# kmaninis/OSVOS-PyTorch

Measured on NVIDIA H100. Metric: frames/sec at 480x854 fwd-only, batch 1 per GPU (OSVOS.forward -> 5 logit maps), higher is better.
Workload: dtype bf16x3 (split-bf16 operands, fp32 accumulate)

## Files before the change

### osvos_pytorch_b200/csrc/conv3x3_halo.cu

```cuda
#include <stdlib.h>
#include <string.h>

#include "conv_common.cuh"

namespace osvos {

constexpr int kHaloRows = kTileH + 2;

template <int BLOCK_N, int PLANES, int PITCH, bool SPLIT>
struct HaloCfg {
  static constexpr int kABoxBytes = kHaloRows * PITCH * 128;
  static constexpr int kAPlaneBytes = (kABoxBytes + 1023) / 1024 * 1024;
  static constexpr int kAStageBytes = PLANES * kAPlaneBytes;
  static constexpr int kAStages = 2;
  static constexpr int kBPlaneBytes = BLOCK_N * 128;
  static constexpr int kBStageBytes = PLANES * kBPlaneBytes;
  static constexpr int kBudget = 225 * 1024 - kAStages * kAStageBytes;
  static constexpr int kBStagesRaw = kBudget / kBStageBytes;
  static constexpr int kBStages = kBStagesRaw > 9 ? 9 : kBStagesRaw;
  static constexpr bool kSplitAcc = SPLIT;
  static_assert(!SPLIT || (PLANES == 2 && BLOCK_N <= 128), "split accumulators need two planes and 2 * BLOCK_N <= 256");
  static constexpr int kAccCols = kSplitAcc ? 2 * BLOCK_N : BLOCK_N;
  static constexpr int kAcc = kAccCols / 2;
  static constexpr int kSmemBytes = kAStages * kAStageBytes + kBStages * kBStageBytes + 1024 + 512;
  static_assert(kBStages >= 2, "weight ring too shallow");
  static_assert(kSmemBytes <= 227 * 1024, "more than the per-CTA shared memory of sm_90");
  static_assert(kSmemBytes + 4096 < (1 << 18), "descriptor start-address field would overflow");
  static_assert(kBStageBytes % 1024 == 0, "B stage must keep 1024-byte alignment");
};

template <int BLOCK_N, int PLANES, int PITCH, bool SPLIT, bool LEAN>
__global__ void __launch_bounds__(kConvThreads, 1)
conv3x3_halo_kernel(const __grid_constant__ CUtensorMap map_x_hi, const __grid_constant__ CUtensorMap map_x_lo,
                    const __grid_constant__ CUtensorMap map_w_hi, const __grid_constant__ CUtensorMap map_w_lo,
                    const ConvParams p) {
  using Cfg = HaloCfg<BLOCK_N, PLANES, PITCH, SPLIT>;
  constexpr int SA = Cfg::kAStages, SB = Cfg::kBStages;

  extern __shared__ uint8_t smem_raw[];
  uint8_t* smem = reinterpret_cast<uint8_t*>((reinterpret_cast<uintptr_t>(smem_raw) + 1023) & ~uintptr_t(1023));
  uint8_t* smem_a = smem;
  uint8_t* smem_b = smem + SA * Cfg::kAStageBytes;
  uint64_t* bars = reinterpret_cast<uint64_t*>(smem_b + SB * Cfg::kBStageBytes);
  uint64_t* a_full = bars;
  uint64_t* a_empty = bars + SA;
  uint64_t* b_full = bars + 2 * SA;
  uint64_t* b_empty = bars + 2 * SA + SB;

  const int warp = threadIdx.x >> 5;
  const int lane = threadIdx.x & 31;

  if (warp == 0 && lane == 0) {
    tma_prefetch_desc(&map_x_hi);
    tma_prefetch_desc(&map_w_hi);
    if (PLANES == 2) {
      tma_prefetch_desc(&map_x_lo);
      tma_prefetch_desc(&map_w_lo);
    }
    for (int i = 0; i < SA; ++i) {
      mbar_init(&a_full[i], 1);
      mbar_init(&a_empty[i], 2);
    }
    for (int i = 0; i < SB; ++i) {
      mbar_init(&b_full[i], 1);
      mbar_init(&b_empty[i], 2);
    }
    fence_barrier_init();
  }
  __syncthreads();
  pdl_wait();
  pdl_launch_dependents();

  if (warp == 0) {
    if (elect_one()) {
      int a_stage = 0, b_stage = 0;
      uint32_t a_phase = 0, b_phase = 0;
      const bool skip_a = (p.ablate & 2) != 0, skip_b = (p.ablate & 1) != 0;
      auto issue_a = [&](int x0, int y0, int img, int kc) {
        mbar_wait(&a_empty[a_stage], a_phase ^ 1);
        if (skip_a) {
          mbar_arrive(&a_full[a_stage]);
        } else {
          uint8_t* st = smem_a + a_stage * Cfg::kAStageBytes;
          mbar_arrive_expect_tx(&a_full[a_stage], PLANES * Cfg::kABoxBytes);
          tma_load_4d(&map_x_hi, &a_full[a_stage], st, kc * kBlockK, x0, y0, img);
          if (PLANES == 2) tma_load_4d(&map_x_lo, &a_full[a_stage], st + Cfg::kAPlaneBytes, kc * kBlockK, x0, y0, img);
        }
        if (++a_stage == SA) {
          a_stage = 0;
          a_phase ^= 1;
        }
      };
      int nb = 0, tx = 0, ty = 0, img = 0;
      const int w_first = static_cast<int>(blockIdx.x), w_stride = static_cast<int>(gridDim.x);
      if (w_first < p.total_tiles) {
        decode_tile(p, w_first, nb, tx, ty, img);
        issue_a(tx * kTileW - 1, ty * kTileH - 1, img, 0);
      }
      for (int tile = w_first; tile < p.total_tiles; tile += w_stride) {
        const bool has_next = tile + w_stride < p.total_tiles;
        int nnb = 0, ntx = 0, nty = 0, nimg = 0;
        if (has_next) decode_tile(p, tile + w_stride, nnb, ntx, nty, nimg);
        const int n0 = nb * BLOCK_N;
        for (int kc = 0; kc < p.k_chunks; ++kc) {
          const int c0 = kc * kBlockK;
#pragma unroll
          for (int tap = 0; tap < 9; ++tap) {
            if (tap == 3) {
              if (kc + 1 < p.k_chunks) issue_a(tx * kTileW - 1, ty * kTileH - 1, img, kc + 1);
              else if (has_next) issue_a(ntx * kTileW - 1, nty * kTileH - 1, nimg, 0);
            }
            mbar_wait(&b_empty[b_stage], b_phase ^ 1);
            if (skip_b) {
              mbar_arrive(&b_full[b_stage]);
            } else {
              uint8_t* st = smem_b + b_stage * Cfg::kBStageBytes;
              mbar_arrive_expect_tx(&b_full[b_stage], Cfg::kBStageBytes);
              tma_load_3d(&map_w_hi, &b_full[b_stage], st, c0, n0, tap);
              if (PLANES == 2) tma_load_3d(&map_w_lo, &b_full[b_stage], st + Cfg::kBPlaneBytes, c0, n0, tap);
            }
            if (++b_stage == SB) {
              b_stage = 0;
              b_phase ^= 1;
            }
          }
        }
        nb = nnb, tx = ntx, ty = nty, img = nimg;
      }
    }
    __syncwarp();
  } else if (warp >= 4) {
    const int wg = (warp - 4) >> 2, wl = warp & 3;
    const bool leader = (threadIdx.x & 127) == 0;
    constexpr uint64_t kDescA = desc_template(16, PITCH * 128, kDescSW128);
    constexpr uint64_t kDescB = desc_template(16, 1024, kDescSW128);
    constexpr uint32_t kLoPlaneA = Cfg::kAPlaneBytes >> 4, kLoPlaneB = Cfg::kBPlaneBytes >> 4;
    const uint32_t smem_a_u32 = smem_u32(smem_a) + wg * 8 * PITCH * 128, smem_b_u32 = smem_u32(smem_b);
    const int k_steps = (p.ablate & 4) ? 0 : p.k_steps;
    float acc[Cfg::kAcc];
    int a_stage = 0, b_stage = 0;
    uint32_t a_phase = 0, b_phase = 0;
    StageRelease pending;
    for (int tile = blockIdx.x; tile < p.total_tiles; tile += gridDim.x) {
#pragma unroll
      for (int i = 0; i < Cfg::kAcc; ++i) acc[i] = 0.f;
      for (int kc = 0; kc < p.k_chunks; ++kc) {
        mbar_wait(&a_full[a_stage], a_phase);
        const uint64_t da0 = kDescA | static_cast<uint64_t>((smem_a_u32 + a_stage * Cfg::kAStageBytes) >> 4);
#pragma unroll
        for (int tap = 0; tap < 9; ++tap) {
          const uint32_t tap_off = static_cast<uint32_t>(((tap / 3) * PITCH + (tap % 3)) * (128 >> 4));
          mbar_wait(&b_full[b_stage], b_phase);
          const uint64_t db_hi = kDescB | static_cast<uint64_t>((smem_b_u32 + b_stage * Cfg::kBStageBytes) >> 4);
          const uint64_t da_hi = da0 + tap_off;
          const uint64_t da_lo = da_hi + kLoPlaneA;
          wgmma_fence();
          auto k_step = [&](int k) {
            if constexpr (Cfg::kSplitAcc) {
              wgmma_bf16<2 * BLOCK_N>(acc, da_hi + 2 * k, db_hi + 2 * k, 1);
              wgmma_bf16<BLOCK_N>(acc, da_lo + 2 * k, db_hi + 2 * k, 1);
            } else if constexpr (PLANES == 2) {
              wgmma_bf16<BLOCK_N>(acc, da_lo + 2 * k, db_hi + 2 * k, 1);
              wgmma_bf16<BLOCK_N>(acc, da_hi + 2 * k, db_hi + kLoPlaneB + 2 * k, 1);
              wgmma_bf16<BLOCK_N>(acc, da_hi + 2 * k, db_hi + 2 * k, 1);
            } else {
              wgmma_bf16<BLOCK_N>(acc, da_hi + 2 * k, db_hi + 2 * k, 1);
            }
          };
          if (k_steps == kBlockK / 16) {
#pragma unroll
            for (int k = 0; k < kBlockK / 16; ++k) k_step(k);
          } else {
            for (int k = 0; k < k_steps; ++k) k_step(k);
          }
          wgmma_commit();
          wgmma_wait<1>();
          pending.release(leader);
          pending.bar_b = &b_empty[b_stage];
          if (tap == 8) pending.bar_a = &a_empty[a_stage];
          if (++b_stage == SB) {
            b_stage = 0;
            b_phase ^= 1;
          }
        }
        if (++a_stage == SA) {
          a_stage = 0;
          a_phase ^= 1;
        }
      }
      wgmma_wait<0>();
      wgmma_fence_operands(acc);
      pending.release(leader);
      conv_epilogue<BLOCK_N, Cfg::kSplitAcc, LEAN>(p, acc, tile, wg, wl, lane);
    }
  }
}

struct HaloSwitches {
  bool lean;
  bool n256;
  bool splitacc128;
};
static bool env_flag(const char* name, bool dflt) {
  const char* e = getenv(name);
  return e == nullptr ? dflt : atoi(e) != 0;
}
static HaloSwitches halo_switches() {
  static HaloSwitches sw;
  static int state = 0;
  if (state != 1) {
    sw.lean = env_flag("OSVOS_HALO_LEAN", true);
    sw.n256 = env_flag("OSVOS_CONV_N256", true);
    sw.splitacc128 = env_flag("OSVOS_SPLITACC128", true);
    state = env_flag("OSVOS_ENV_RELOAD", false) ? 2 : 1;
  }
  return sw;
}

template <int BLOCK_N, int PLANES, int PITCH, bool SPLIT = (PLANES == 2 && BLOCK_N <= 128), bool LEAN = false>
static int launch_halo(const osvos_conv3x3_args* a, cudaStream_t stream) {
  using Cfg = HaloCfg<BLOCK_N, PLANES, PITCH, SPLIT>;
  ConvParams p;
  fill_conv_params(p, a, BLOCK_N);
  const int sms = device_sm_count();
  CUtensorMap mx_hi, mx_lo, mw_hi, mw_lo;
  {
    const uint64_t dims[4] = {(uint64_t)a->cin, (uint64_t)a->w, (uint64_t)a->h, (uint64_t)a->n};
    const uint64_t strides[3] = {(uint64_t)a->cin * 2, (uint64_t)a->w * a->cin * 2,
                                 (uint64_t)a->h * a->w * a->cin * 2};
    const uint32_t box[4] = {kBlockK, PITCH, kHaloRows, 1};
    int rc = encode_tensor_map(&mx_hi, CU_TENSOR_MAP_DATA_TYPE_BFLOAT16, 2, 4, a->x_hi, dims, strides, box,
                               CU_TENSOR_MAP_SWIZZLE_128B);
    if (rc) return rc;
    rc = encode_tensor_map(&mx_lo, CU_TENSOR_MAP_DATA_TYPE_BFLOAT16, 2, 4, PLANES == 2 ? a->x_lo : a->x_hi, dims,
                           strides, box, CU_TENSOR_MAP_SWIZZLE_128B);
    if (rc) return rc;
  }
  int rc = encode_weight_maps(&mw_hi, &mw_lo, a, BLOCK_N);
  if (rc) return rc;
  auto kern = conv3x3_halo_kernel<BLOCK_N, PLANES, PITCH, SPLIT, LEAN>;
  static uint64_t attr_done = 0;
  OSVOS_CHECK_CUDA(ensure_dynamic_smem(kern, Cfg::kSmemBytes, &attr_done));
  const int grid = p.total_tiles < sms ? p.total_tiles : sms;
  OSVOS_CHECK_CUDA(launch_pdl(kern, dim3(grid), dim3(kConvThreads), Cfg::kSmemBytes, stream, mx_hi, mx_lo,
                              mw_hi, mw_lo, p));
  return OSVOS_OK;
}

template <int PITCH>
static int dispatch_halo(const osvos_conv3x3_args* a, cudaStream_t stream) {
  const bool fast = (a->flags & OSVOS_FLAG_FAST) != 0;
  const HaloSwitches sw = halo_switches();
  if (a->cout == 16) return fast ? launch_halo<16, 1, PITCH>(a, stream) : launch_halo<16, 2, PITCH>(a, stream);
  const bool lean = sw.lean && !fast && !(a->flags & OSVOS_FLAG_RELU_MASK) && a->colsum == nullptr && a->y_f32 == nullptr &&
                    a->pq == nullptr && a->k_valid == 0;
  if (a->cout == 64) {
    if (lean) return launch_halo<64, 2, PITCH, true, true>(a, stream);
    return fast ? launch_halo<64, 1, PITCH>(a, stream) : launch_halo<64, 2, PITCH>(a, stream);
  }
  const int m_tiles = ((a->w + kTileW - 1) / kTileW) * ((a->h + kTileH - 1) / kTileH) * a->n;
  const int sms = device_sm_count();
  const long tiles128 = static_cast<long>(m_tiles) * (a->cout / 128);
  const long waves128 = (tiles128 + sms - 1) / sms;
  const long waves256 = (static_cast<long>(m_tiles) * (a->cout / 256) + sms - 1) / sms;
  if (waves128 == 1 && tiles128 * 5 <= static_cast<long>(sms) * 3) {
    if (lean) return launch_halo<64, 2, PITCH, true, true>(a, stream);
    return fast ? launch_halo<64, 1, PITCH>(a, stream) : launch_halo<64, 2, PITCH>(a, stream);
  }
  const bool prefer256 = fast ? waves256 * 1100 < waves128 * 700 : waves256 * 2200 < waves128 * 1000;
  if (a->cout % 256 == 0 && prefer256 && sw.n256)
    return fast ? launch_halo<256, 1, PITCH>(a, stream) : launch_halo<256, 2, PITCH>(a, stream);
  if (fast) return launch_halo<128, 1, PITCH>(a, stream);
  if (!sw.splitacc128) return launch_halo<128, 2, PITCH, false>(a, stream);
  if (lean) return launch_halo<128, 2, PITCH, true, true>(a, stream);
  return launch_halo<128, 2, PITCH>(a, stream);
}

int conv3x3_halo_dispatch(const osvos_conv3x3_args* a, cudaStream_t stream) {
  return dispatch_halo<10>(a, stream);
}

static int check_conv_args(const osvos_conv3x3_args* a) {
  OSVOS_CHECK_ARG(a != nullptr);
  OSVOS_CHECK_ARG(a->n > 0 && a->h > 0 && a->w > 0);
  OSVOS_CHECK_ARG(a->cin >= 64 && a->cin % 64 == 0);
  OSVOS_CHECK_ARG(a->cout == 2 || a->cout == 16 || a->cout == 64 || (a->cout > 0 && a->cout % 128 == 0));
  OSVOS_CHECK_ARG(a->cout != 2 || (a->pq != nullptr && a->y_hi == nullptr && a->y_f32 == nullptr && a->pool_hi == nullptr &&
                                   a->colsum == nullptr && !(a->flags & (OSVOS_FLAG_RELU | OSVOS_FLAG_RELU_MASK)) &&
                                   a->k_valid == 0));
  OSVOS_CHECK_ARG(a->x_hi != nullptr && a->w_packed != nullptr);
  OSVOS_CHECK_ARG((a->flags & OSVOS_FLAG_FAST) || a->x_lo != nullptr);
  OSVOS_CHECK_ARG(a->y_hi != nullptr || a->y_f32 != nullptr || a->pq != nullptr || a->pool_hi != nullptr);
  OSVOS_CHECK_ARG(!(a->flags & OSVOS_FLAG_RELU_MASK) || a->mask_hi != nullptr);
  OSVOS_CHECK_ARG(a->pq == nullptr || a->cout == 2 || (a->cout == 16 && a->proj_w != nullptr));
  OSVOS_CHECK_ARG((a->pool_hi == nullptr && a->colsum == nullptr) || a->cout >= 64);
  OSVOS_CHECK_ARG((reinterpret_cast<uintptr_t>(a->x_hi) & 15) == 0);
  OSVOS_CHECK_ARG((reinterpret_cast<uintptr_t>(a->w_packed) & 15) == 0);
  OSVOS_CHECK_ARG((reinterpret_cast<uintptr_t>(a->bias) & 15) == 0);
  if (a->cout >= 64) {
    const uintptr_t bf16_planes = reinterpret_cast<uintptr_t>(a->y_hi) | reinterpret_cast<uintptr_t>(a->y_lo) |
                                  reinterpret_cast<uintptr_t>(a->pool_hi) | reinterpret_cast<uintptr_t>(a->pool_lo) |
                                  reinterpret_cast<uintptr_t>(a->mask_hi);
    OSVOS_CHECK_ARG((bf16_planes & 3) == 0);
    OSVOS_CHECK_ARG((reinterpret_cast<uintptr_t>(a->y_f32) & 7) == 0);
  }
  OSVOS_CHECK_ARG(a->k_valid >= 0 && a->k_valid <= 64 && a->k_valid % 16 == 0);
  return OSVOS_OK;
}

}

using namespace osvos;

extern "C" int osvos_side_folded_multi(const osvos_conv3x3_args* args, int count, osvos_stream_t stream_) {
  OSVOS_CHECK_ARG(args != nullptr && count > 0 && count <= 4);
  const osvos_conv3x3_args* order[4];
  for (int k = 0; k < count; ++k) {
    int rc = check_conv_args(&args[k]);
    if (rc) return rc;
    OSVOS_CHECK_ARG(args[k].cout == 2);
    OSVOS_CHECK_ARG((args[k].flags & OSVOS_FLAG_FAST) == (args[0].flags & OSVOS_FLAG_FAST));
    order[k] = &args[k];
  }
  for (int i = 1; i < count; ++i)
    for (int j = i; j > 0 && order[j]->cin > order[j - 1]->cin; --j) {
      const osvos_conv3x3_args* t = order[j];
      order[j] = order[j - 1];
      order[j - 1] = t;
    }
  return side_conv_multi_dispatch(order, count, static_cast<cudaStream_t>(stream_));
}

extern "C" int osvos_conv3x3(const osvos_conv3x3_args* a, osvos_stream_t stream_) {
  int rc = check_conv_args(a);
  if (rc) return rc;
  cudaStream_t stream = static_cast<cudaStream_t>(stream_);
  if (a->cout == 2) return side_conv_dispatch(a, stream);
  if (a->cout == 16 && a->y_hi == nullptr && !(a->flags & OSVOS_FLAG_RELU_MASK) && a->colsum == nullptr) {
    static int generic = -1;
    if (generic < 0) {
      const char* side = getenv("OSVOS_SIDE_IMPL");
      generic = (side != nullptr && strcmp(side, "generic") == 0) ? 1 : 0;
    }
    if (!generic) return side_conv_dispatch(a, stream);
  }
  return conv3x3_halo_dispatch(a, stream);
}
```

### osvos_pytorch_b200/csrc/conv_common.cuh

```cuda
#pragma once
#include <stdlib.h>

#include "common.cuh"
#include "ptx.cuh"

namespace osvos {

constexpr int kTileW = 8;
constexpr int kTileH = 16;
constexpr int kBlockM = 128;
constexpr int kBlockK = 64;
constexpr int kConvThreads = 384;
constexpr int kABytes = kBlockM * kBlockK * 2;

struct ConvParams {
  const float* bias;
  __nv_bfloat16* y_hi;
  __nv_bfloat16* y_lo;
  float* y_f32;
  const __nv_bfloat16* mask_hi;
  const float* proj_w;
  const float* proj_b;
  float* pq;
  __nv_bfloat16* pool_hi;
  __nv_bfloat16* pool_lo;
  float* colsum;
  int n, h, w, cin, cout;
  int tiles_x, tiles_y, n_blocks, total_tiles, k_chunks;
  int k_steps;
  int flags;
  int ablate;
};

__device__ __forceinline__ void decode_tile(const ConvParams& p, int tile, int& nb, int& tx, int& ty, int& img) {
  nb = tile % p.n_blocks;
  int m = tile / p.n_blocks;
  tx = m % p.tiles_x;
  m /= p.tiles_x;
  ty = m % p.tiles_y;
  img = m / p.tiles_y;
}

__device__ __forceinline__ uint32_t sw128_offset(int row, int chunk) { return row * 128 + ((chunk ^ (row & 7)) << 4); }

__device__ __forceinline__ void split_pack2(float a, float b, uint32_t& hi, uint32_t& lo) {
  asm("cvt.rn.bf16x2.f32 %0, %1, %2;" : "=r"(hi) : "f"(b), "f"(a));
  const float ra = a - __uint_as_float(hi << 16);
  const float rb = b - __uint_as_float(hi & 0xFFFF0000u);
  asm("cvt.rn.bf16x2.f32 %0, %1, %2;" : "=r"(lo) : "f"(rb), "f"(ra));
}

template <int BLOCK_N, bool SPLIT_ACC, bool LEAN = false>
__device__ __forceinline__ void conv_epilogue(const ConvParams& p, const float* acc, int tile, int wg, int wl, int lane) {
  int nb, tx, ty, img;
  decode_tile(p, tile, nb, tx, ty, img);
  const int lx = lane >> 2;
  const int x = tx * kTileW + lx;
  const int y0 = ty * kTileH + wg * 8 + wl * 2;
  const bool va = (y0 < p.h) && (x < p.w), vb = (y0 + 1 < p.h) && (x < p.w);
  const bool relu = (p.flags & OSVOS_FLAG_RELU) != 0;
  const bool masked = !LEAN && (p.flags & OSVOS_FLAG_RELU_MASK) != 0;
  const bool store_ok = !(p.ablate & 8);
  const size_t pix[2] = {(static_cast<size_t>(img) * p.h + y0) * p.w + x, (static_cast<size_t>(img) * p.h + y0 + 1) * p.w + x};
  const bool valid[2] = {va, vb};
  const int oh = (p.h + 1) >> 1, ow = (p.w + 1) >> 1;
  const bool pool_writer = va && !(lx & 1) && store_ok;
  const size_t opix = (static_cast<size_t>(img) * oh + (y0 >> 1)) * ow + (x >> 1);
  float sp[2] = {0.f, 0.f}, sq[2] = {0.f, 0.f};
#pragma unroll
  for (int j = 0; j < BLOCK_N / 8; ++j) {
    const int c = 8 * j + 2 * (lane & 3);
    const int ch = nb * BLOCK_N + c;
    const float2 b = p.bias ? __ldg(reinterpret_cast<const float2*>(p.bias + ch)) : make_float2(0.f, 0.f);
    float f[2][2];
#pragma unroll
    for (int h = 0; h < 2; ++h) {
#pragma unroll
      for (int e = 0; e < 2; ++e) {
        float v = e ? b.y : b.x;
        v += acc[4 * j + 2 * h + e];
        if (SPLIT_ACC) v += acc[BLOCK_N / 2 + 4 * j + 2 * h + e];
        f[h][e] = relu ? fmaxf(v, 0.f) : v;
      }
    }
#pragma unroll
    for (int h = 0; h < 2; ++h) {
      if (!LEAN && masked && valid[h]) {
        const uint32_t m = __ldg(reinterpret_cast<const unsigned int*>(p.mask_hi + pix[h] * p.cout + ch));
        if (!(bf16_lo_to_float(m) > 0.f)) f[h][0] = 0.f;
        if (!(bf16_hi_to_float(m) > 0.f)) f[h][1] = 0.f;
      }
      if (valid[h] && store_ok) {
        if (!LEAN && p.y_f32) *reinterpret_cast<float2*>(p.y_f32 + pix[h] * p.cout + ch) = make_float2(f[h][0], f[h][1]);
        if (p.y_hi) {
          uint32_t hi, lo;
          split_pack2(f[h][0], f[h][1], hi, lo);
          *reinterpret_cast<uint32_t*>(p.y_hi + pix[h] * p.cout + ch) = hi;
          if (p.y_lo) *reinterpret_cast<uint32_t*>(p.y_lo + pix[h] * p.cout + ch) = lo;
        }
      }
      if (!LEAN && BLOCK_N == 16 && p.pq) {
        sp[h] = fmaf(f[h][0], __ldg(p.proj_w + c), fmaf(f[h][1], __ldg(p.proj_w + c + 1), sp[h]));
        sq[h] = fmaf(f[h][0], __ldg(p.proj_w + 16 + c), fmaf(f[h][1], __ldg(p.proj_w + 16 + c + 1), sq[h]));
      }
    }
    if (!LEAN && p.colsum) {
      float s0 = (va ? f[0][0] : 0.f) + (vb ? f[1][0] : 0.f);
      float s1 = (va ? f[0][1] : 0.f) + (vb ? f[1][1] : 0.f);
#pragma unroll
      for (int o = 4; o <= 16; o <<= 1) {
        s0 += __shfl_xor_sync(0xffffffffu, s0, o);
        s1 += __shfl_xor_sync(0xffffffffu, s1, o);
      }
      if (lane < 4) {
        atomicAdd(p.colsum + ch, s0);
        atomicAdd(p.colsum + ch + 1, s1);
      }
    }
    if (p.pool_hi) {
      float m0 = fmaxf(va ? f[0][0] : -INFINITY, vb ? f[1][0] : -INFINITY);
      float m1 = fmaxf(va ? f[0][1] : -INFINITY, vb ? f[1][1] : -INFINITY);
      m0 = fmaxf(m0, __shfl_xor_sync(0xffffffffu, m0, 4));
      m1 = fmaxf(m1, __shfl_xor_sync(0xffffffffu, m1, 4));
      if (pool_writer) {
        uint32_t hi, lo;
        split_pack2(m0, m1, hi, lo);
        *reinterpret_cast<uint32_t*>(p.pool_hi + opix * p.cout + ch) = hi;
        if (p.pool_lo) *reinterpret_cast<uint32_t*>(p.pool_lo + opix * p.cout + ch) = lo;
      }
    }
  }
  if (!LEAN && BLOCK_N == 16 && p.pq) {
#pragma unroll
    for (int h = 0; h < 2; ++h) {
      sp[h] += __shfl_xor_sync(0xffffffffu, sp[h], 1);
      sp[h] += __shfl_xor_sync(0xffffffffu, sp[h], 2);
      sq[h] += __shfl_xor_sync(0xffffffffu, sq[h], 1);
      sq[h] += __shfl_xor_sync(0xffffffffu, sq[h], 2);
      if ((lane & 3) == 0 && valid[h] && store_ok)
        *reinterpret_cast<float2*>(p.pq + pix[h] * 2) = make_float2(sp[h] + (p.proj_b ? __ldg(p.proj_b) : 0.f), sq[h]);
    }
  }
}


static inline void fill_conv_params(ConvParams& p, const osvos_conv3x3_args* a, int block_n) {
  p.bias = a->bias;
  p.y_hi = static_cast<__nv_bfloat16*>(a->y_hi);
  p.y_lo = static_cast<__nv_bfloat16*>(a->y_lo);
  p.y_f32 = a->y_f32;
  p.mask_hi = static_cast<const __nv_bfloat16*>(a->mask_hi);
  p.proj_w = a->proj_w;
  p.proj_b = a->proj_b;
  p.pq = a->pq;
  p.pool_hi = static_cast<__nv_bfloat16*>(a->pool_hi);
  p.pool_lo = static_cast<__nv_bfloat16*>(a->pool_lo);
  p.colsum = a->colsum;
  p.n = a->n;
  p.h = a->h;
  p.w = a->w;
  p.cin = a->cin;
  p.cout = a->cout;
  p.tiles_x = (a->w + kTileW - 1) / kTileW;
  p.tiles_y = (a->h + kTileH - 1) / kTileH;
  p.n_blocks = a->cout / block_n;
  p.total_tiles = p.tiles_x * p.tiles_y * a->n * p.n_blocks;
  p.k_chunks = a->cin / kBlockK;
  p.k_steps = (a->k_valid > 0 && a->k_valid < kBlockK) ? (a->k_valid + 15) / 16 : kBlockK / 16;
  p.flags = a->flags;
  {
    static int ablate = -1;
    if (ablate < 0) {
      const char* e = getenv("OSVOS_ABLATE");
      ablate = e ? atoi(e) : 0;
    }
    p.ablate = ablate;
  }
}

static inline int encode_weight_maps(CUtensorMap* hi, CUtensorMap* lo, const osvos_conv3x3_args* a, int block_n) {
  const size_t plane = static_cast<size_t>(9) * a->cout * a->cin;
  const uint64_t dims[3] = {(uint64_t)a->cin, (uint64_t)a->cout, 9};
  const uint64_t strides[2] = {(uint64_t)a->cin * 2, (uint64_t)a->cout * a->cin * 2};
  const uint32_t box[3] = {kBlockK, (uint32_t)block_n, 1};
  const __nv_bfloat16* wp = static_cast<const __nv_bfloat16*>(a->w_packed);
  int rc = encode_tensor_map(hi, CU_TENSOR_MAP_DATA_TYPE_BFLOAT16, 2, 3, wp, dims, strides, box,
                             CU_TENSOR_MAP_SWIZZLE_128B);
  if (rc) return rc;
  return encode_tensor_map(lo, CU_TENSOR_MAP_DATA_TYPE_BFLOAT16, 2, 3, wp + plane, dims, strides, box,
                           CU_TENSOR_MAP_SWIZZLE_128B);
}

int conv_first_tc_launch(const float* x, const float* w_oihw, const float* bias, void* y_hi, void* y_lo, int n, int h,
                         int w, int flags, cudaStream_t stream);
int side_conv_dispatch(const osvos_conv3x3_args* a, cudaStream_t stream);
int side_conv_multi_dispatch(const osvos_conv3x3_args* const* args, int count, cudaStream_t stream);
int conv3x3_halo_dispatch(const osvos_conv3x3_args* a, cudaStream_t stream);

}
```

### osvos_pytorch_b200/csrc/ptx.cuh

```cuda
#pragma once
#include <cuda.h>
#include <cuda_runtime.h>
#include <stdint.h>

#include "wgmma.cuh"

namespace osvos {

#ifndef OSVOS_SPIN_LIMIT
#define OSVOS_SPIN_LIMIT (1u << 26)
#endif

__device__ __forceinline__ uint32_t smem_u32(const void* p) {
  return static_cast<uint32_t>(__cvta_generic_to_shared(p));
}
__device__ __forceinline__ uint32_t lane_id() { return threadIdx.x & 31; }

__device__ __forceinline__ bool elect_one() {
  uint32_t pred = 0;
  asm volatile(
      "{\n\t.reg .pred P;\n\t"
      "elect.sync _|P, 0xffffffff;\n\t"
      "selp.u32 %0, 1, 0, P;\n\t}\n"
      : "=r"(pred));
  return pred != 0;
}

__device__ __forceinline__ void pdl_wait() { asm volatile("griddepcontrol.wait;" ::: "memory"); }
__device__ __forceinline__ void pdl_launch_dependents() { asm volatile("griddepcontrol.launch_dependents;" ::: "memory"); }

__device__ __forceinline__ void mbar_init(uint64_t* bar, uint32_t count) {
  asm volatile("mbarrier.init.shared::cta.b64 [%0], %1;" ::"r"(smem_u32(bar)), "r"(count) : "memory");
}
__device__ __forceinline__ void fence_barrier_init() {
  asm volatile("fence.mbarrier_init.release.cluster;" ::: "memory");
}
__device__ __forceinline__ void fence_proxy_async_smem() {
  asm volatile("fence.proxy.async.shared::cta;" ::: "memory");
}
__device__ __forceinline__ void mbar_arrive_expect_tx(uint64_t* bar, uint32_t bytes) {
  asm volatile("mbarrier.arrive.expect_tx.shared::cta.b64 _, [%0], %1;" ::"r"(smem_u32(bar)), "r"(bytes)
               : "memory");
}
__device__ __forceinline__ void mbar_arrive(uint64_t* bar) {
  asm volatile("mbarrier.arrive.shared::cta.b64 _, [%0];" ::"r"(smem_u32(bar)) : "memory");
}
__device__ __forceinline__ bool mbar_try_wait(uint64_t* bar, uint32_t parity) {
  uint32_t ok;
  asm volatile(
      "{\n\t.reg .pred P;\n\t"
      "mbarrier.try_wait.parity.shared::cta.b64 P, [%1], %2;\n\t"
      "selp.u32 %0, 1, 0, P;\n\t}\n"
      : "=r"(ok)
      : "r"(smem_u32(bar)), "r"(parity)
      : "memory");
  return ok != 0;
}
__device__ __forceinline__ uint32_t ld_acquire_gpu_u32(const unsigned int* p) {
  uint32_t v;
  asm volatile("ld.acquire.gpu.global.u32 %0, [%1];" : "=r"(v) : "l"(p) : "memory");
  return v;
}
__device__ __forceinline__ void red_release_gpu_add_u32(unsigned int* p, uint32_t v) {
  asm volatile("red.release.gpu.global.add.u32 [%0], %1;" ::"l"(p), "r"(v) : "memory");
}
__device__ __forceinline__ void st_relaxed_gpu_u32(unsigned int* p, uint32_t v) {
  asm volatile("st.relaxed.gpu.global.u32 [%0], %1;" ::"l"(p), "r"(v) : "memory");
}

__device__ __forceinline__ void mbar_wait(uint64_t* bar, uint32_t parity) {
  uint32_t spins = 0;
  while (!mbar_try_wait(bar, parity)) {
    if (++spins > OSVOS_SPIN_LIMIT) __trap();
  }
}

__device__ __forceinline__ void cp_async_8_zfill(void* dst, const void* src, uint32_t src_bytes) {
  asm volatile("cp.async.ca.shared.global [%0], [%1], 8, %2;" ::"r"(smem_u32(dst)), "l"(src), "r"(src_bytes) : "memory");
}
__device__ __forceinline__ void cp_async_mbar_arrive_noinc(uint64_t* bar) {
  asm volatile("cp.async.mbarrier.arrive.noinc.shared::cta.b64 [%0];" ::"r"(smem_u32(bar)) : "memory");
}

__device__ __forceinline__ void tma_prefetch_desc(const CUtensorMap* m) {
  asm volatile("prefetch.tensormap [%0];" ::"l"(reinterpret_cast<uint64_t>(m)) : "memory");
}
__device__ __forceinline__ void tma_load_4d(const CUtensorMap* m, uint64_t* bar, void* dst, int c0, int c1, int c2,
                                            int c3) {
  asm volatile(
      "cp.async.bulk.tensor.4d.shared::cluster.global.mbarrier::complete_tx::bytes"
      " [%0], [%1, {%3, %4, %5, %6}], [%2];"
      ::"r"(smem_u32(dst)), "l"(reinterpret_cast<uint64_t>(m)), "r"(smem_u32(bar)), "r"(c0), "r"(c1), "r"(c2),
      "r"(c3)
      : "memory");
}
__device__ __forceinline__ void tma_load_5d(const CUtensorMap* m, uint64_t* bar, void* dst, int c0, int c1, int c2,
                                            int c3, int c4) {
  asm volatile(
      "cp.async.bulk.tensor.5d.shared::cluster.global.mbarrier::complete_tx::bytes"
      " [%0], [%1, {%3, %4, %5, %6, %7}], [%2];"
      ::"r"(smem_u32(dst)), "l"(reinterpret_cast<uint64_t>(m)), "r"(smem_u32(bar)), "r"(c0), "r"(c1), "r"(c2),
      "r"(c3), "r"(c4)
      : "memory");
}
__device__ __forceinline__ void tma_load_2d(const CUtensorMap* m, uint64_t* bar, void* dst, int c0, int c1) {
  asm volatile(
      "cp.async.bulk.tensor.2d.shared::cluster.global.mbarrier::complete_tx::bytes"
      " [%0], [%1, {%3, %4}], [%2];"
      ::"r"(smem_u32(dst)), "l"(reinterpret_cast<uint64_t>(m)), "r"(smem_u32(bar)), "r"(c0), "r"(c1)
      : "memory");
}
__device__ __forceinline__ void tma_load_3d(const CUtensorMap* m, uint64_t* bar, void* dst, int c0, int c1, int c2) {
  asm volatile(
      "cp.async.bulk.tensor.3d.shared::cluster.global.mbarrier::complete_tx::bytes"
      " [%0], [%1, {%3, %4, %5}], [%2];"
      ::"r"(smem_u32(dst)), "l"(reinterpret_cast<uint64_t>(m)), "r"(smem_u32(bar)), "r"(c0), "r"(c1), "r"(c2)
      : "memory");
}
__device__ __forceinline__ void tma_store_4d(const CUtensorMap* m, const void* src, int c0, int c1, int c2, int c3) {
  asm volatile("cp.async.bulk.tensor.4d.global.shared::cta.bulk_group [%0, {%2, %3, %4, %5}], [%1];"
               ::"l"(reinterpret_cast<uint64_t>(m)), "r"(smem_u32(src)), "r"(c0), "r"(c1), "r"(c2), "r"(c3)
               : "memory");
}
__device__ __forceinline__ void tma_store_commit() { asm volatile("cp.async.bulk.commit_group;" ::: "memory"); }
template <int N>
__device__ __forceinline__ void tma_store_wait_read() {
  asm volatile("cp.async.bulk.wait_group.read %0;" ::"n"(N) : "memory");
}
template <int N>
__device__ __forceinline__ void tma_store_wait_all() {
  asm volatile("cp.async.bulk.wait_group %0;" ::"n"(N) : "memory");
}

constexpr uint64_t kDescSW128 = 1ull << 62;
constexpr uint64_t kDescSW64 = 2ull << 62;
__host__ __device__ constexpr uint64_t desc_template(uint32_t lbo_bytes, uint32_t sbo_bytes, uint64_t layout) {
  return (static_cast<uint64_t>((lbo_bytes >> 4) & 0x3FFF) << 16) | (static_cast<uint64_t>((sbo_bytes >> 4) & 0x3FFF) << 32) |
         layout;
}
__device__ __forceinline__ uint64_t make_smem_desc(const void* p, uint32_t lbo_bytes, uint32_t sbo_bytes, uint64_t layout) {
  return desc_template(lbo_bytes, sbo_bytes, layout) | static_cast<uint64_t>((smem_u32(p) >> 4) & 0x3FFF);
}

__device__ __forceinline__ void named_bar_sync(int id, int nthreads) {
  asm volatile("bar.sync %0, %1;" ::"r"(id), "r"(nthreads) : "memory");
}

struct StageRelease {
  uint64_t* bar_b = nullptr;
  uint64_t* bar_a = nullptr;
  __device__ __forceinline__ void release(bool leader) {
    if (leader) {
      if (bar_b) mbar_arrive(bar_b);
      if (bar_a) mbar_arrive(bar_a);
    }
    bar_b = bar_a = nullptr;
  }
};

}
```

Baseline: 578.0.

## Add ping-pong warpgroup schedule for halo conv with register reallocation

Adds a ping-pong variant where each of the two consumer warpgroups owns a whole tile (both M halves) and alternates tiles, using named barriers so one warpgroup's epilogue overlaps the other's MMA mainloop. Producer warps give up registers through setmaxnreg so consumers can hold the doubled accumulator. Ring stage and phase are recomputed from the tile sequence, and barrier reader counts drop to one. It is selected when there are more than twice as many tiles as SMs. The cost is higher register pressure and possible spills or ordering bugs in the shared A/B ring.

```diff
diff --git a/osvos_pytorch_b200/csrc/conv3x3_halo.cu b/osvos_pytorch_b200/csrc/conv3x3_halo.cu
--- a/osvos_pytorch_b200/csrc/conv3x3_halo.cu
+++ b/osvos_pytorch_b200/csrc/conv3x3_halo.cu
@@ -29,13 +29,15 @@
   static_assert(kBStageBytes % 1024 == 0, "B stage must keep 1024-byte alignment");
 };
 
-template <int BLOCK_N, int PLANES, int PITCH, bool SPLIT, bool LEAN>
+template <int BLOCK_N, int PLANES, int PITCH, bool SPLIT, bool LEAN, bool PINGPONG>
 __global__ void __launch_bounds__(kConvThreads, 1)
 conv3x3_halo_kernel(const __grid_constant__ CUtensorMap map_x_hi, const __grid_constant__ CUtensorMap map_x_lo,
                     const __grid_constant__ CUtensorMap map_w_hi, const __grid_constant__ CUtensorMap map_w_lo,
                     const ConvParams p) {
   using Cfg = HaloCfg<BLOCK_N, PLANES, PITCH, SPLIT>;
   constexpr int SA = Cfg::kAStages, SB = Cfg::kBStages;
+  constexpr int kHalves = PINGPONG ? 2 : 1;
+  static_assert(!PINGPONG || kHalves * Cfg::kAcc <= 128, "a ping-pong warpgroup holds the whole tile's accumulator");
 
   extern __shared__ uint8_t smem_raw[];
   uint8_t* smem = reinterpret_cast<uint8_t*>((reinterpret_cast<uintptr_t>(smem_raw) + 1023) & ~uintptr_t(1023));
@@ -57,13 +59,14 @@
       tma_prefetch_desc(&map_x_lo);
       tma_prefetch_desc(&map_w_lo);
     }
+    constexpr uint32_t kReaders = PINGPONG ? 1 : 2;
     for (int i = 0; i < SA; ++i) {
       mbar_init(&a_full[i], 1);
-      mbar_init(&a_empty[i], 2);
+      mbar_init(&a_empty[i], kReaders);
     }
     for (int i = 0; i < SB; ++i) {
       mbar_init(&b_full[i], 1);
-      mbar_init(&b_empty[i], 2);
+      mbar_init(&b_empty[i], kReaders);
     }
     fence_barrier_init();
   }
@@ -71,7 +74,9 @@
   pdl_wait();
   pdl_launch_dependents();
 
-  if (warp == 0) {
+  if (warp < 4) {
+    if (PINGPONG) setmaxnreg_dec<40>();
+    if (warp != 0) return;
     if (elect_one()) {
       int a_stage = 0, b_stage = 0;
       uint32_t a_phase = 0, b_phase = 0;
@@ -129,21 +134,31 @@
       }
     }
     __syncwarp();
-  } else if (warp >= 4) {
+  } else {
+    if (PINGPONG) setmaxnreg_inc<232>();
     const int wg = (warp - 4) >> 2, wl = warp & 3;
     const bool leader = (threadIdx.x & 127) == 0;
     constexpr uint64_t kDescA = desc_template(16, PITCH * 128, kDescSW128);
     constexpr uint64_t kDescB = desc_template(16, 1024, kDescSW128);
     constexpr uint32_t kLoPlaneA = Cfg::kAPlaneBytes >> 4, kLoPlaneB = Cfg::kBPlaneBytes >> 4;
-    const uint32_t smem_a_u32 = smem_u32(smem_a) + wg * 8 * PITCH * 128, smem_b_u32 = smem_u32(smem_b);
+    constexpr uint32_t kHalfA = (8 * PITCH * 128) >> 4;
+    const uint32_t smem_a_u32 = smem_u32(smem_a) + (PINGPONG ? 0 : wg * 8 * PITCH * 128), smem_b_u32 = smem_u32(smem_b);
     const int k_steps = (p.ablate & 4) ? 0 : p.k_steps;
-    float acc[Cfg::kAcc];
-    int a_stage = 0, b_stage = 0;
-    uint32_t a_phase = 0, b_phase = 0;
+    float acc[kHalves][Cfg::kAcc];
     StageRelease pending;
-    for (int tile = blockIdx.x; tile < p.total_tiles; tile += gridDim.x) {
-#pragma unroll
-      for (int i = 0; i < Cfg::kAcc; ++i) acc[i] = 0.f;
+    constexpr int kOwners = PINGPONG ? 2 : 1;
+    for (int k = PINGPONG ? wg : 0;; k += kOwners) {
+      const int tile = static_cast<int>(blockIdx.x) + k * static_cast<int>(gridDim.x);
+      if (tile >= p.total_tiles) break;
+      const bool has_next = tile + static_cast<int>(gridDim.x) < p.total_tiles;
+      const int a_seq = k * p.k_chunks, b_seq = 9 * a_seq;
+      int a_stage = a_seq % SA, b_stage = b_seq % SB;
+      uint32_t a_phase = (a_seq / SA) & 1, b_phase = (b_seq / SB) & 1;
+      if (PINGPONG && k > 0) named_bar_sync(1 + wg, 256);
+#pragma unroll
+      for (int h = 0; h < kHalves; ++h)
+#pragma unroll
+        for (int i = 0; i < Cfg::kAcc; ++i) acc[h][i] = 0.f;
       for (int kc = 0; kc < p.k_chunks; ++kc) {
         mbar_wait(&a_full[a_stage], a_phase);
         const uint64_t da0 = kDescA | static_cast<uint64_t>((smem_a_u32 + a_stage * Cfg::kAStageBytes) >> 4);
@@ -151,27 +166,31 @@
         for (int tap = 0; tap < 9; ++tap) {
           const uint32_t tap_off = static_cast<uint32_t>(((tap / 3) * PITCH + (tap % 3)) * (128 >> 4));
           mbar_wait(&b_full[b_stage], b_phase);
+          if (PINGPONG && tap == 8 && kc == p.k_chunks - 1 && has_next) named_bar_arrive(1 + (wg ^ 1), 256);
           const uint64_t db_hi = kDescB | static_cast<uint64_t>((smem_b_u32 + b_stage * Cfg::kBStageBytes) >> 4);
-          const uint64_t da_hi = da0 + tap_off;
-          const uint64_t da_lo = da_hi + kLoPlaneA;
           wgmma_fence();
-          auto k_step = [&](int k) {
-            if constexpr (Cfg::kSplitAcc) {
-              wgmma_bf16<2 * BLOCK_N>(acc, da_hi + 2 * k, db_hi + 2 * k, 1);
-              wgmma_bf16<BLOCK_N>(acc, da_lo + 2 * k, db_hi + 2 * k, 1);
-            } else if constexpr (PLANES == 2) {
-              wgmma_bf16<BLOCK_N>(acc, da_lo + 2 * k, db_hi + 2 * k, 1);
-              wgmma_bf16<BLOCK_N>(acc, da_hi + 2 * k, db_hi + kLoPlaneB + 2 * k, 1);
-              wgmma_bf16<BLOCK_N>(acc, da_hi + 2 * k, db_hi + 2 * k, 1);
+#pragma unroll
+          for (int h = 0; h < kHalves; ++h) {
+            const uint64_t da_hi = da0 + h * kHalfA + tap_off;
+            const uint64_t da_lo = da_hi + kLoPlaneA;
+            auto k_step = [&](int ks) {
+              if constexpr (Cfg::kSplitAcc) {
+                wgmma_bf16<2 * BLOCK_N>(acc[h], da_hi + 2 * ks, db_hi + 2 * ks, 1);
+                wgmma_bf16<BLOCK_N>(acc[h], da_lo + 2 * ks, db_hi + 2 * ks, 1);
+              } else if constexpr (PLANES == 2) {
+                wgmma_bf16<BLOCK_N>(acc[h], da_lo + 2 * ks, db_hi + 2 * ks, 1);
+                wgmma_bf16<BLOCK_N>(acc[h], da_hi + 2 * ks, db_hi + kLoPlaneB + 2 * ks, 1);
+                wgmma_bf16<BLOCK_N>(acc[h], da_hi + 2 * ks, db_hi + 2 * ks, 1);
+              } else {
+                wgmma_bf16<BLOCK_N>(acc[h], da_hi + 2 * ks, db_hi + 2 * ks, 1);
+              }
+            };
+            if (k_steps == kBlockK / 16) {
+#pragma unroll
+              for (int ks = 0; ks < kBlockK / 16; ++ks) k_step(ks);
             } else {
-              wgmma_bf16<BLOCK_N>(acc, da_hi + 2 * k, db_hi + 2 * k, 1);
+              for (int ks = 0; ks < k_steps; ++ks) k_step(ks);
             }
-          };
-          if (k_steps == kBlockK / 16) {
-#pragma unroll
-            for (int k = 0; k < kBlockK / 16; ++k) k_step(k);
-          } else {
-            for (int k = 0; k < k_steps; ++k) k_step(k);
           }
           wgmma_commit();
           wgmma_wait<1>();
@@ -189,9 +208,12 @@
         }
       }
       wgmma_wait<0>();
-      wgmma_fence_operands(acc);
+#pragma unroll
+      for (int h = 0; h < kHalves; ++h) wgmma_fence_operands(acc[h]);
       pending.release(leader);
-      conv_epilogue<BLOCK_N, Cfg::kSplitAcc, LEAN>(p, acc, tile, wg, wl, lane);
+#pragma unroll
+      for (int h = 0; h < kHalves; ++h)
+        conv_epilogue<BLOCK_N, Cfg::kSplitAcc, LEAN>(p, acc[h], tile, PINGPONG ? h : wg, wl, lane);
     }
   }
 }
@@ -238,10 +260,13 @@
   }
   int rc = encode_weight_maps(&mw_hi, &mw_lo, a, BLOCK_N);
   if (rc) return rc;
-  auto kern = conv3x3_halo_kernel<BLOCK_N, PLANES, PITCH, SPLIT, LEAN>;
-  static uint64_t attr_done = 0;
-  OSVOS_CHECK_CUDA(ensure_dynamic_smem(kern, Cfg::kSmemBytes, &attr_done));
   const int grid = p.total_tiles < sms ? p.total_tiles : sms;
+  constexpr bool kCanPingPong = BLOCK_N == 64 || BLOCK_N == 128;
+  const bool pingpong = kCanPingPong && p.total_tiles > 2 * sms;
+  auto kern = pingpong ? conv3x3_halo_kernel<BLOCK_N, PLANES, PITCH, SPLIT && BLOCK_N == 64, LEAN, kCanPingPong>
+                       : conv3x3_halo_kernel<BLOCK_N, PLANES, PITCH, SPLIT, LEAN, false>;
+  static uint64_t attr_done[2] = {0, 0};
+  OSVOS_CHECK_CUDA(ensure_dynamic_smem(kern, Cfg::kSmemBytes, &attr_done[pingpong]));
   OSVOS_CHECK_CUDA(launch_pdl(kern, dim3(grid), dim3(kConvThreads), Cfg::kSmemBytes, stream, mx_hi, mx_lo,
                               mw_hi, mw_lo, p));
   return OSVOS_OK;
diff --git a/osvos_pytorch_b200/csrc/conv_common.cuh b/osvos_pytorch_b200/csrc/conv_common.cuh
--- a/osvos_pytorch_b200/csrc/conv_common.cuh
+++ b/osvos_pytorch_b200/csrc/conv_common.cuh
@@ -52,6 +52,7 @@
 
 template <int BLOCK_N, bool SPLIT_ACC, bool LEAN = false>
 __device__ __forceinline__ void conv_epilogue(const ConvParams& p, const float* acc, int tile, int wg, int wl, int lane) {
+  if (p.ablate & 16) return;
   int nb, tx, ty, img;
   decode_tile(p, tile, nb, tx, ty, img);
   const int lx = lane >> 2;
diff --git a/osvos_pytorch_b200/csrc/ptx.cuh b/osvos_pytorch_b200/csrc/ptx.cuh
--- a/osvos_pytorch_b200/csrc/ptx.cuh
+++ b/osvos_pytorch_b200/csrc/ptx.cuh
@@ -145,6 +145,14 @@
 __device__ __forceinline__ void named_bar_sync(int id, int nthreads) {
   asm volatile("bar.sync %0, %1;" ::"r"(id), "r"(nthreads) : "memory");
 }
+__device__ __forceinline__ void named_bar_arrive(int id, int nthreads) {
+  asm volatile("bar.arrive %0, %1;" ::"r"(id), "r"(nthreads) : "memory");
+}
+
+template <int N>
+__device__ __forceinline__ void setmaxnreg_dec() { asm volatile("setmaxnreg.dec.sync.aligned.u32 %0;" ::"n"(N)); }
+template <int N>
+__device__ __forceinline__ void setmaxnreg_inc() { asm volatile("setmaxnreg.inc.sync.aligned.u32 %0;" ::"n"(N)); }
 
 struct StageRelease {
   uint64_t* bar_b = nullptr;
```

Result: faster. 597.0, median of 6 (+3.3%).
